# multicom-toolbox/Chromosome3D

Measured on AMD Instinct MI355X. Metric: SA-steps/sec (replica-steps/s, 20 replicas of chr1_500kb in all: 20 per GPU, weak scaling; regions of 20 steps inside the first 2172 of the schedule's 5172: MD and FIRE steps in front of the final minimisation); wall-clock per chromosome, higher is better.
Workload: dtype f32

## Files before the change

chromosome3d_amd/csrc/c3d_batch_main.cpp:

```cpp
#include <dirent.h>
#include <sys/stat.h>

#include <algorithm>
#include <atomic>
#include <chrono>
#include <condition_variable>
#include <cstdio>
#include <cstdlib>
#include <cstring>
#include <mutex>
#include <string>
#include <thread>
#include <vector>

#include "../../include/c3d.h"

namespace {

struct Job {
    std::string path, id, chrom;
    double cost = 0;
    int device = -1, half = -1;
    bool ok = false;
    std::string summary;
};
struct Options {
    std::string out;
    double K = 11, alpha = 0.5, gtol = 1e-2;
    int final_min = 1;
    bool lbfgs = false;
    int models = 20, min_steps = 3000;
    unsigned long long seed = 82364ULL;
    bool violations = false;
};
std::mutex g_print;
bool g_timeline = false;
double g_t0 = 0;
bool g_warm = true;
bool g_pair = true;

struct XcdBroker {
    std::mutex mu;
    std::condition_variable cv;
    bool busy[2] = {false, false};
    int waiting_full = 0;
    int acquire(bool half) {
        std::unique_lock<std::mutex> lk(mu);
        if (!half) {
            ++waiting_full;
            cv.wait(lk, [&] { return !busy[0] && !busy[1]; });
            --waiting_full;
            busy[0] = busy[1] = true;
            return -1;
        }
        cv.wait(lk, [&] { return waiting_full == 0 && (!busy[0] || !busy[1]); });
        const int h = busy[0] ? 1 : 0;
        busy[h] = true;
        return h;
    }
    void release(int h) {
        { std::lock_guard<std::mutex> lk(mu); if (h < 0) busy[0] = busy[1] = false; else busy[h] = false; }
        cv.notify_all();
    }
};
double now_s() { return std::chrono::duration<double>(std::chrono::steady_clock::now().time_since_epoch()).count(); }

#define TRY(call)                                                                                  \
    do {                                                                                           \
        if ((call) != C3D_OK) { job.summary = std::string(#call) + ": " + c3d_last_error(); return false; } \
    } while (0)

bool solve_one(c3d_ctx* ctx, const Options& o, Job& job, XcdBroker& gpu) {
    const double t0 = now_s();
    const std::string dir = o.out + "/" + job.chrom;
    mkdir(dir.c_str(), 0755);
    c3d_model model;
    c3d_default_model(&model);
    TRY(c3d_set_model(ctx, &model));
    double* IF = nullptr;
    int n = 0, R = 0;
    TRY(c3d_parse_if_file(job.path.c_str(), &IF, &n));
    std::vector<double> if_copy(IF, IF + (size_t)n * n);
    c3d_free(IF);
    if (n > C3D_MAX_BEADS_DEFAULT && n <= C3D_MAX_BEADS_LIMIT) TRY(c3d_set_option(ctx, "max_beads", n));
    TRY(c3d_set_if_matrix(ctx, if_copy.data(), n, o.alpha, o.K));
    const double t_k1 = now_s();
    std::vector<int32_t> d10((size_t)n * n);
    TRY(c3d_get_dist10(ctx, d10.data()));
    const std::string tbl = dir + "/contact.tbl";
    TRY(c3d_write_front_half(d10.data(), n, model.min_sep, (dir + "/" + job.id + ".dist").c_str(), (dir + "/" + job.id + ".rr").c_str(),
                             tbl.c_str(), &R));
    {
        FILE* fa = fopen((dir + "/" + job.id + ".fasta").c_str(), "w");
        if (!fa) { job.summary = "cannot write " + job.id + ".fasta"; return false; }
        fprintf(fa, ">%s\n%s\n", job.id.c_str(), std::string((size_t)n, 'M').c_str());
        if (fclose(fa) != 0) { job.summary = "cannot write " + job.id + ".fasta"; return false; }
    }
    std::vector<c3d_stage> stages(c3d_default_schedule(nullptr, 0, o.min_steps));
    c3d_default_schedule(stages.data(), (int)stages.size(), o.min_steps);
    if (o.lbfgs) stages.back().kind = 8;
    c3d_fire_params fire;
    c3d_default_fire(&fire);
    TRY(c3d_set_option(ctx, "final_minimiser", o.final_min));
    TRY(c3d_set_schedule(ctx, stages.data(), (int)stages.size(), &fire, (float)o.gtol, 250));
    bool half = false;
    if (g_pair && n <= 270) {
        TRY(c3d_set_option(ctx, "cluster_xcd_base", 0));
        TRY(c3d_set_option(ctx, "cluster_xcd_count", 4));
        TRY(c3d_init_replicas(ctx, o.models, o.seed, 0));
        double ok = 0;
        c3d_get_stat(ctx, "cluster_ok", &ok);
        half = ok != 0;
    }
    if (!half) {
        TRY(c3d_set_option(ctx, "cluster_xcd_base", 0));
        TRY(c3d_set_option(ctx, "cluster_xcd_count", 8));
        TRY(c3d_init_replicas(ctx, o.models, o.seed, 0));
    }
    const double t_front = now_s();
    double t_anneal0 = t_front;
    {
        struct Hold {
            XcdBroker& b; int h;
            ~Hold() { b.release(h); }
        } hold{gpu, gpu.acquire(half)};
        if (half) TRY(c3d_set_option(ctx, "cluster_xcd_base", 4 * hold.h));
        t_anneal0 = now_s();
        TRY(c3d_run(ctx));
        job.half = half ? hold.h : -1;
    }
    const double t_run = now_s();
    double ms = 0;
    long steps = 0, launches = 0;
    c3d_last_timing(ctx, &ms, &steps, &launches);
    const int M = o.models;
    std::vector<float> xyz((size_t)M * n * 3);
    std::vector<double> en((size_t)M * 3), rho(M);
    std::vector<int32_t> rank(M);
    TRY(c3d_get_coords(ctx, xyz.data()));
    TRY(c3d_get_energies(ctx, en.data()));
    TRY(c3d_rank(ctx, rank.data()));
    std::vector<int32_t> sats(M);
    std::vector<double> devs(M);
    TRY(c3d_score_replicas(ctx, if_copy.data(), 3, sats.data(), devs.data(), rho.data()));
    const double t_score = now_s();
    const int Rt = R;
    struct FileCloser {
        FILE* f;
        ~FileCloser() { if (f) fclose(f); }
    } lgc{fopen((o.out + "/" + job.chrom + ".log").c_str(), "w")};
    FILE* const lg = lgc.f;
    if (!lg) { job.summary = "cannot write the log"; return false; }
    fprintf(lg, "L          : %d\nRestraints : %d lines in tbl file\n\nNOE_SATISFIED(+-0.5A)  SUM_OF_DEVIATIONS>= 0.2  PDB\n", n, R);
    std::vector<std::string> names(M);
    std::vector<int32_t> vri, vrj, vrt;
    remove((dir + "/model_info.log").c_str());
    for (int k = M - 1; k >= 0; --k) {
        const int r = rank[k];
        char name[96];
        snprintf(name, sizeof name, "%s_%d.pdb", job.id.c_str(), r + 1);
        names[r] = dir + "/" + name;
        TRY(c3d_write_pdb(names[r].c_str(), xyz.data() + (size_t)r * n * 3, n, en[3 * r], en[3 * r + 1], en[3 * r + 2], name));
        int sat = sats[r];
        double dev = devs[r];
        if (o.violations) {
            if (vri.empty()) {
                int32_t *pi = nullptr, *pj = nullptr, *pt = nullptr;
                int Rr = 0;
                TRY(c3d_read_tbl(tbl.c_str(), &pi, &pj, &pt, &Rr));
                vri.assign(pi, pi + Rr); vrj.assign(pj, pj + Rr); vrt.assign(pt, pt + Rr);
                c3d_free(pi); c3d_free(pj); c3d_free(pt);
                remove((dir + "/contact_violation.txt").c_str());
            }
            TRY(c3d_write_violations(xyz.data() + (size_t)r * n * 3, n, (int)vri.size(), vri.data(), vrj.data(), vrt.data(), 0.5, ("./" + std::string(name)).c_str(),
                                     "contact.tbl", (dir + "/contact_violation.txt").c_str(), &sat, &dev));
        }
        char cnt[48], sd[48];
        snprintf(cnt, sizeof cnt, "%d/%d", sat, Rt);
        snprintf(sd, sizeof sd, "%.2f", dev);
        std::string base(name);
        base.resize(base.size() - 4);
        fprintf(lg, "%-9s             %-9s                %-25s\n", cnt, sd, base.c_str());
    }
    for (int k = M - 1; k >= 0; --k) TRY(c3d_shape_pdb(names[rank[k]].c_str(), names[rank[k]].c_str(), (dir + "/model_info.log").c_str()));
    fprintf(lg, "\n");
    for (int k = 0; k < M && k < 5; ++k) {
        char dst[96];
        snprintf(dst, sizeof dst, "%s_model%d.pdb", job.id.c_str(), k + 1);
        fprintf(lg, "model%d.pdb <= %s\n", k + 1, names[rank[k]].c_str());
        if (rename(names[rank[k]].c_str(), (dir + "/" + dst).c_str()) != 0) { job.summary = "rename failed"; return false; }
    }
    lgc.f = nullptr;
    if (fclose(lg) != 0) { job.summary = "cannot write the log"; return false; }
    char buf[512];
    const double t_end = now_s();
    snprintf(buf, sizeof buf, "%-14s N=%4d R=%6d  %2d models  best: replica %2d  E_noe %12.1f  Spearman(IF,1/d) %.4f  anneal %6.1f ms (%ld steps)  "
                              "end-to-end %.2f s  GPU %d%s  [phases: parse+K1 %.3f, front-half files+start structures %.3f, anneal %.3f, read-back+rank+Spearman %.3f, "
                              "PDB+assessment+shaping %.3f s]",
             job.chrom.c_str(), n, R, M, rank[0] + 1, en[3 * rank[0]], -rho[rank[0]], ms, steps, t_end - t0, job.device, job.half < 0 ? "" : (job.half ? " XCDs 4-7" : " XCDs 0-3"), t_k1 - t0, t_front - t_k1,
             t_run - t_anneal0, t_score - t_run, t_end - t_score);
    job.summary = buf;
    if (g_timeline) {
        std::lock_guard<std::mutex> lk(g_print);
        fprintf(stderr, "timeline %-12s N=%4d start %.4f parsed+K1 %.4f front %.4f got-GPU %.4f annealed %.4f scored %.4f end %.4f%s\n", job.chrom.c_str(), n,
                t0 - g_t0, t_k1 - g_t0, t_front - g_t0, t_anneal0 - g_t0, t_run - g_t0, t_score - g_t0, t_end - g_t0, job.half < 0 ? "" : (job.half ? " half 1" : " half 0"));
    }
    return true;
}

void collect(const std::string& arg, const std::string& pattern, std::vector<Job>& jobs) {
    struct stat st;
    if (stat(arg.c_str(), &st) != 0) { fprintf(stderr, "c3d_batch: %s not found\n", arg.c_str()); exit(2); }
    std::vector<std::string> files;
    if (S_ISDIR(st.st_mode)) {
        DIR* d = opendir(arg.c_str());
        while (dirent* e = d ? readdir(d) : nullptr) {
            const std::string f = e->d_name;
            if (f.size() > 11 && f.compare(f.size() - 11, 11, "_matrix.txt") == 0) files.push_back(arg + "/" + f);
        }
        if (d) closedir(d);
    } else {
        files.push_back(arg);
    }
    std::sort(files.begin(), files.end());
    for (const std::string& f : files) {
        if (!pattern.empty() && f.find(pattern) == std::string::npos) continue;
        Job j;
        j.path = f;
        std::string base = f.substr(f.find_last_of('/') + 1);
        j.id = base.size() > 4 && base.compare(base.size() - 4, 4, ".txt") == 0 ? base.substr(0, base.size() - 4) : base;
        j.chrom = j.id.size() > 7 && j.id.compare(j.id.size() - 7, 7, "_matrix") == 0 ? j.id.substr(0, j.id.size() - 7) : j.id;
        stat(f.c_str(), &st);
        j.cost = (double)st.st_size;
        jobs.push_back(j);
    }
}

}

int main(int argc, char** argv) {
    setenv("HSA_DISABLE_COREDUMP_ON_EXCEPTION", "1", 0);
    Options o;
    std::vector<std::string> inputs;
    std::string pattern;
    int devices = -1, lanes = 3, map_to = -1;
    for (int a = 1; a < argc; ++a) {
        const std::string s = argv[a];
        auto next = [&](const char* what) -> const char* {
            if (a + 1 >= argc) { fprintf(stderr, "c3d_batch: %s needs a value\n", what); exit(2); }
            return argv[++a];
        };
        if (s == "--out" || s == "-o") o.out = next("--out");
        else if (s == "--devices") devices = atoi(next("--devices"));
        else if (s == "--pair") g_pair = atoi(next("--pair")) != 0;
        else if (s == "--order") g_warm = std::string(next("--order")) != "lpt";
        else if (s == "--map-devices-to") map_to = atoi(next("--map-devices-to"));
        else if (s == "--lanes") lanes = std::max(1, std::min(8, atoi(next("--lanes"))));
        else if (s == "-m") o.models = atoi(next("-m"));
        else if (s == "-k") o.K = atof(next("-k"));
        else if (s == "-a") o.alpha = atof(next("-a"));
        else if (s == "--seed") o.seed = strtoull(next("--seed"), nullptr, 10);
        else if (s == "--min-steps") o.min_steps = atoi(next("--min-steps"));
        else if (s == "--gtol") o.gtol = atof(next("--gtol"));
        else if (s == "--final-minimiser") o.final_min = atoi(next("--final-minimiser"));
        else if (s == "--lbfgs") o.lbfgs = true;
        else if (s == "--pattern") pattern = next("--pattern");
        else if (s == "--violations") o.violations = true;
        else if (s == "-h" || s == "--help") { printf("usage: c3d_batch <dir | matrix files...> --out <root> [--devices N] [--lanes 3] [-m 20] [-k 11] [-a 0.5] [--seed S] [--min-steps 3000] [--gtol 1e-2] [--final-minimiser 1] [--lbfgs] [--pattern text] [--violations] [--pair 1] [--order warm|lpt] [--map-devices-to P (rehearsal)]\n"); return 0; }
        else inputs.push_back(s);
    }
    if (o.out.empty() || inputs.empty() || o.models < 1) { fprintf(stderr, "c3d_batch: need input matrices and --out <root> (see --help)\n"); return 2; }
    std::vector<Job> jobs;
    for (const std::string& in : inputs) collect(in, pattern, jobs);
    if (jobs.empty()) { fprintf(stderr, "c3d_batch: no *_matrix.txt found\n"); return 2; }
    const int ndev = c3d_device_count();
    if (ndev < 1) { fprintf(stderr, "c3d_batch: no HIP device visible: libc3d has no CPU fallback\n"); return 1; }
    if (map_to >= ndev) { fprintf(stderr, "c3d_batch: --map-devices-to %d: this machine has %d device(s)\n", map_to, ndev); return 2; }
    if (map_to >= 0) { if (devices < 1) devices = 1; if (devices > 64) devices = 64; }
    else if (devices < 1 || devices > ndev) devices = ndev;
    mkdir(o.out.c_str(), 0755);
    std::vector<size_t> order(jobs.size());
    for (size_t k = 0; k < order.size(); ++k) order[k] = k;
    std::stable_sort(order.begin(), order.end(), [&](size_t a, size_t b) { return jobs[a].cost > jobs[b].cost; });
    std::vector<double> load(devices, 0.0);
    std::vector<std::vector<size_t>> mine(devices);
    for (size_t k : order) {
        const int g = (int)(std::min_element(load.begin(), load.end()) - load.begin());
        jobs[k].device = g;
        load[g] += jobs[k].cost;
        mine[g].push_back(k);
    }
    if (g_warm && lanes > 1)
        for (int g = 0; g < devices; ++g) {
            std::vector<size_t>& q = mine[g];
            const size_t small = std::min((size_t)(lanes - 1), q.size() > 1 ? q.size() - 1 : 0);
            if (small == 0) continue;
            std::vector<size_t> head(1, q[0]);
            for (size_t k = 0; k < small; ++k) head.push_back(q[q.size() - 1 - k]);
            head.insert(head.end(), q.begin() + 1, q.end() - small);
            q.swap(head);
        }
    const double t0 = now_s();
    g_t0 = t0;
    g_timeline = getenv("C3D_BATCH_TIMELINE") != nullptr;
    std::atomic<int> failed{0};
    std::vector<std::thread> workers;
    std::vector<XcdBroker> gpu_mu(devices);
    std::vector<std::atomic<size_t>> next_job(devices);
    std::vector<std::atomic<int>> lanes_up(devices);
    for (int g = 0; g < devices; ++g) { next_job[g] = 0; lanes_up[g] = 0; }
    for (int g = 0; g < devices; ++g)
      for (int lane = 0; lane < lanes; ++lane)
        workers.emplace_back([&, g]() {
            c3d_ctx* ctx = nullptr;
            const int phys = map_to >= 0 ? map_to : g;
            if (c3d_create(phys, &ctx) != C3D_OK) {
                std::lock_guard<std::mutex> lk(g_print);
                fprintf(stderr, "c3d_batch: GPU %d: %s\n", g, c3d_last_error());
                return;
            }
            ++lanes_up[g];
            if (g_timeline) { std::lock_guard<std::mutex> lk(g_print); fprintf(stderr, "timeline lane of GPU %d has its context at %.4f\n", g, now_s() - g_t0); }
            for (;;) {
                const size_t at = next_job[g]++;
                if (at >= mine[g].size()) break;
                Job& job = jobs[mine[g][at]];
                job.ok = solve_one(ctx, o, job, gpu_mu[map_to >= 0 ? 0 : g]);
                std::lock_guard<std::mutex> lk(g_print);
                if (job.ok) printf("%s\n", job.summary.c_str());
                else { printf("FAILED: %s (%s)\n", job.chrom.c_str(), job.summary.c_str()); ++failed; }
                fflush(stdout);
            }
            c3d_destroy(ctx);
        });
    for (std::thread& w : workers) w.join();
    for (int g = 0; g < devices; ++g) {
        if (lanes_up[g] > 0) continue;
        for (size_t at = 0; at < mine[g].size(); ++at) {
            printf("FAILED: %s (no context on GPU %d)\n", jobs[mine[g][at]].chrom.c_str(), g);
            ++failed;
        }
    }
    printf("c3d_batch: %zu matrices x %d models on %d GPU(s), %d lane(s) each, in %.2f s, %d failed; models under %s/<chromosome>/<ID>_model1..5.pdb\n", jobs.size(),
           o.models, devices, lanes, now_s() - t0, failed.load(), o.out.c_str());
    return failed.load() ? 1 : 0;
}
```

chromosome3d_amd/csrc/c3d_solve_main.cpp:

```cpp
#include <sys/stat.h>

#include <chrono>
#include <cstdio>
#include <cstdlib>
#include <cstring>
#include <string>
#include <vector>

#include "../../include/c3d.h"

static void usage() {
    fprintf(stderr,
            "usage: c3d_solve (--if <IF matrix> | --tbl <contact.tbl> --n <beads>) --out <dir> [--id <ID>]\n"
            "                 [-k <K=11>] [-a <alpha=0.5>] [-m <models=20>] [--seed <82364>] [--first-replica <0>]\n"
            "                 [--device <0>] [--min-steps <3000>] [--gtol <1e-2>] [--final-minimiser <1>] [--lbfgs] [--embed] [--no-graph] [--quiet]\n"
            "                 [--precision <32>   64: anneal with the fp64 step kernels (the reference's arithmetic; with --lbfgs the final stage is\n"
            "                                     L-BFGS in fp64); beyond 2560 beads the fp64 target matrix takes 8 n^2 bytes more]\n"
            "                 [--embed-max-beads <4549>   the largest matrix --embed takes, up to 16384 (memory: 8 n^2 bytes + 4 n^2 per replica of a batch)]\n"
            "                 [--seq <one-letter residue codes | @fasta file>   residue names of the models (default: all MET)]\n"
            "                 [--similarity <path>   after the solve, the replicas against one another: one row `a b spearman rmsd` per ordered pair of\n"
            "                                        replica ids (Spearman and scaled RMSD of the pair distances, computed on the device)]\n"
            "                 [--accepted   also write <ID>a_<k>.pdb beside every <ID>_<k>.pdb, as CNS does for structures it accepts]\n");
}

#define CHECK(call)                                                              \
    do {                                                                         \
        int rc__ = (call);                                                       \
        if (rc__ != C3D_OK) {                                                    \
            fprintf(stderr, "c3d_solve: %s failed (%d): %s\n", #call, rc__, c3d_last_error()); \
            return fail_exit(out_dir);                                           \
        }                                                                        \
    } while (0)

static int fail_exit(const std::string& out_dir) {
    if (!out_dir.empty()) {
        const std::string a = out_dir + "/iam.running", b = out_dir + "/iam.failed";
        if (rename(a.c_str(), b.c_str()) != 0) { FILE* f = fopen(b.c_str(), "w"); if (f) fclose(f); }
    }
    fprintf(stderr, "ERROR! Final structures not found!\nC3D FAILED!\n");
    return 1;
}

static double now_s() { return std::chrono::duration<double>(std::chrono::steady_clock::now().time_since_epoch()).count(); }

int main(int argc, char** argv) {
    setenv("HSA_DISABLE_COREDUMP_ON_EXCEPTION", "1", 0);
    const double t_start = now_s();
    std::string if_path, tbl_path, out_dir, id, seq_arg, similarity_path;
    double K = 11, alpha = 0.5, gtol = 1e-2;
    int final_min = 1;
    int lbfgs = 0;
    int models = 20, device = 0, n_beads = 0, min_steps = 3000, use_graph = 1, quiet = 0, embed = 0, embed_max_beads = 0, accepted = 0, precision = 32;
    unsigned long long seed = 82364ULL;
    unsigned first_rep = 0;
    for (int a = 1; a < argc; ++a) {
        const std::string s = argv[a];
        auto next = [&](const char* what) -> const char* {
            if (a + 1 >= argc) { fprintf(stderr, "c3d_solve: %s needs a value\n", what); exit(2); }
            return argv[++a];
        };
        if (s == "--if" || s == "-i" || s == "-if") if_path = next("--if");
        else if (s == "--tbl") tbl_path = next("--tbl");
        else if (s == "--n") n_beads = atoi(next("--n"));
        else if (s == "--out" || s == "-o") out_dir = next("--out");
        else if (s == "--id") id = next("--id");
        else if (s == "-k") K = atof(next("-k"));
        else if (s == "-a") alpha = atof(next("-a"));
        else if (s == "-m") models = atoi(next("-m"));
        else if (s == "--seed") seed = strtoull(next("--seed"), nullptr, 10);
        else if (s == "--first-replica") first_rep = (unsigned)strtoul(next("--first-replica"), nullptr, 10);
        else if (s == "--device") device = atoi(next("--device"));
        else if (s == "--min-steps") min_steps = atoi(next("--min-steps"));
        else if (s == "--gtol") gtol = atof(next("--gtol"));
        else if (s == "--final-minimiser") final_min = atoi(next("--final-minimiser"));
        else if (s == "--lbfgs") lbfgs = 1;
        else if (s == "--embed") embed = 1;
        else if (s == "--embed-max-beads") embed_max_beads = atoi(next("--embed-max-beads"));
        else if (s == "--precision") precision = atoi(next("--precision"));
        else if (s == "--no-graph") use_graph = 0;
        else if (s == "--quiet") quiet = 1;
        else if (s == "--accepted") accepted = 1;
        else if (s == "--seq") seq_arg = next("--seq");
        else if (s == "--similarity") similarity_path = next("--similarity");
        else if (s == "-h" || s == "--help") { usage(); return 0; }
        else { fprintf(stderr, "c3d_solve: unknown option %s\n", s.c_str()); usage(); return 2; }
    }
    if (out_dir.empty() || (if_path.empty() == tbl_path.empty()) || models < 1) { usage(); return 2; }
    if (id.empty()) {
        std::string base = if_path.empty() ? std::string("model") : if_path.substr(if_path.find_last_of('/') + 1);
        if (base.size() > 4 && base.substr(base.size() - 4) == ".txt") base.resize(base.size() - 4);
        id = base;
    }
    if (!seq_arg.empty()) {
        std::string letters = seq_arg;
        if (seq_arg[0] == '@') {
            FILE* f = fopen(seq_arg.c_str() + 1, "r");
            if (!f) { fprintf(stderr, "c3d_solve: cannot read %s\n", seq_arg.c_str() + 1); return 2; }
            letters.clear();
            char line[4096];
            while (fgets(line, sizeof line, f)) if (line[0] != '>') letters += line;
            fclose(f);
        }
        c3d_set_residue_sequence(letters.c_str());
    }
    mkdir(out_dir.c_str(), 0755);
    { FILE* f = fopen((out_dir + "/iam.running").c_str(), "w"); if (!f) { fprintf(stderr, "c3d_solve: cannot write into %s\n", out_dir.c_str()); return 1; } fclose(f); }
    remove((out_dir + "/iam.failed").c_str());

    c3d_ctx* ctx = nullptr;
    CHECK(c3d_create(device, &ctx));
    const double t_ctx = now_s();
    c3d_model model;
    c3d_default_model(&model);
    CHECK(c3d_set_model(ctx, &model));

    int n = 0, R = 0;
    std::vector<int32_t> ri, rj, rt;
    double* IF = nullptr;
    if (!if_path.empty()) {
        CHECK(c3d_parse_if_file(if_path.c_str(), &IF, &n));
        if (n > C3D_MAX_BEADS_DEFAULT && n <= C3D_MAX_BEADS_LIMIT) CHECK(c3d_set_option(ctx, "max_beads", n));
        CHECK(c3d_set_if_matrix(ctx, IF, n, alpha, K));
        std::vector<int32_t> d10((size_t)n * n);
        CHECK(c3d_get_dist10(ctx, d10.data()));
        CHECK(c3d_write_front_half(d10.data(), n, model.min_sep, (out_dir + "/" + id + ".dist").c_str(),
                                   (out_dir + "/" + id + ".rr").c_str(), (out_dir + "/contact.tbl").c_str(), &R));
        if (!quiet) printf("L          : %d\nRestraints : %d lines in tbl file\n", n, R);
    } else {
        int32_t *pi = nullptr, *pj = nullptr, *pt = nullptr;
        CHECK(c3d_read_tbl(tbl_path.c_str(), &pi, &pj, &pt, &R));
        ri.assign(pi, pi + R); rj.assign(pj, pj + R); rt.assign(pt, pt + R);
        c3d_free(pi); c3d_free(pj); c3d_free(pt);
        n = n_beads;
        for (int k = 0; k < R; ++k) { if (ri[k] > n) n = ri[k]; if (rj[k] > n) n = rj[k]; }
        if (n > C3D_MAX_BEADS_DEFAULT && n <= C3D_MAX_BEADS_LIMIT) CHECK(c3d_set_option(ctx, "max_beads", n));
        CHECK(c3d_set_restraints(ctx, n, R, ri.data(), rj.data(), rt.data()));
    }

    const double t_front = now_s();
    std::vector<c3d_stage> stages(c3d_default_schedule(nullptr, 0, min_steps));
    c3d_default_schedule(stages.data(), (int)stages.size(), min_steps);
    if (lbfgs) stages.back().kind = 8;
    c3d_fire_params fire;
    c3d_default_fire(&fire);
    CHECK(c3d_set_option(ctx, "final_minimiser", final_min));
    CHECK(c3d_set_schedule(ctx, stages.data(), (int)stages.size(), &fire, (float)gtol, 250));
    CHECK(c3d_set_option(ctx, "use_graph", use_graph));
    if (precision != 32) {
        if (lbfgs) CHECK(c3d_set_option(ctx, "f64_lbfgs", 1));
        CHECK(c3d_set_option(ctx, "precision", precision));
        if (n > C3D_F64_MAX_BEADS_DEFAULT && n <= C3D_F64_MAX_BEADS_LIMIT) CHECK(c3d_set_option(ctx, "f64_max_beads", n));
    }
    CHECK(c3d_init_replicas(ctx, models, seed, first_rep));
    if (embed_max_beads) CHECK(c3d_set_option(ctx, "embed_max_beads", embed_max_beads));
    if (embed) CHECK(c3d_embed_replicas(ctx, 50));
    CHECK(c3d_run(ctx));
    const double t_run = now_s();

    std::vector<float> xyz((size_t)models * n * 3);
    std::vector<double> en((size_t)models * 3);
    CHECK(c3d_get_coords(ctx, xyz.data()));
    CHECK(c3d_get_energies(ctx, en.data()));
    for (int r = 0; r < models; ++r) {
        char name[64];
        snprintf(name, sizeof name, "%s_%u.pdb", id.c_str(), first_rep + (unsigned)r + 1u);
        CHECK(c3d_write_pdb((out_dir + "/" + name).c_str(), xyz.data() + (size_t)r * n * 3, n, en[3 * r], en[3 * r + 1],
                            en[3 * r + 2], name));
        if (accepted) {
            snprintf(name, sizeof name, "%sa_%u.pdb", id.c_str(), first_rep + (unsigned)r + 1u);
            CHECK(c3d_write_pdb((out_dir + "/" + name).c_str(), xyz.data() + (size_t)r * n * 3, n, en[3 * r], en[3 * r + 1],
                                en[3 * r + 2], name));
        }
    }
    if (!similarity_path.empty()) {
        std::vector<double> rho((size_t)models * models), rmsd((size_t)models * models);
        CHECK(c3d_compare_replicas(ctx, nullptr, 0, rho.data(), rmsd.data()));
        FILE* f = fopen(similarity_path.c_str(), "w");
        if (!f) { fprintf(stderr, "c3d_solve: cannot write %s\n", similarity_path.c_str()); return fail_exit(out_dir); }
        fprintf(f, "# replica_a replica_b spearman rmsd   (pair distances of a scaled onto b's; replica r is %s_<r+1>.pdb)\n", id.c_str());
        for (int a = 0; a < models; ++a)
            for (int b = 0; b < models; ++b)
                if (a != b) fprintf(f, "%u %u %.5f %.5f\n", first_rep + (unsigned)a, first_rep + (unsigned)b, rho[(size_t)a * models + b], rmsd[(size_t)a * models + b]);
        fclose(f);
    }
    double ms = 0;
    long steps = 0, launches = 0;
    c3d_last_timing(ctx, &ms, &steps, &launches);
    if (!quiet) {
        printf(accepted ? "trial and accepted structures written.\n" : "trial structures written.\n");
        printf("c3d_solve: %d beads, %d restraints, %d models, %ld SA steps/model in %.1f ms on device %d (%.3g replica-steps/s)\n",
               n, R, models, steps, ms, device, ms > 0 ? 1e3 * (double)steps * models / ms : 0.0);
        if (IF) {
            std::vector<double> rho(models);
            if (c3d_score_replicas(ctx, IF, 3, nullptr, nullptr, rho.data()) == C3D_OK)
                for (int r = 0; r < models; ++r)
                    printf("  model %2u  E_noe %14.2f  Spearman(IF,d) %.4f\n", first_rep + r + 1, en[3 * r], rho[r]);
            else fprintf(stderr, "c3d_solve: models not scored: %s\n", c3d_last_error());
        }
    }
    if (!quiet)
        printf("c3d_solve wall: device init %.3f s, parse + K1 + front-half files %.3f s, anneal (incl. graph build) %.3f s, "
               "read-back + PDB + scoring %.3f s, total %.3f s\n", t_ctx - t_start, t_front - t_ctx, t_run - t_front, now_s() - t_run,
               now_s() - t_start);
    if (IF) c3d_free(IF);
    c3d_destroy(ctx);
    remove((out_dir + "/iam.running").c_str());
    return 0;
}
```

Measured before the change: 4.736 million.

## Overlap host-side parsing, front-half file writes and PDB output with GPU work

Adds a small host task pool and look-ahead parser so the interaction matrix is parsed ahead of time, the front-half files (.dist/.rr/.tbl/.fasta) are written on a helper thread while annealing runs, and per-model PDB writing and shape analysis run in parallel. The goal is to hide host I/O and parsing latency behind device work and each other. The metric counts replica-steps per second inside the annealing phase, so host-side overlap may not affect it, and the extra threads add scheduling complexity and more error-handling paths.

```diff
diff --git a/chromosome3d_amd/csrc/c3d_batch_main.cpp b/chromosome3d_amd/csrc/c3d_batch_main.cpp
--- a/chromosome3d_amd/csrc/c3d_batch_main.cpp
+++ b/chromosome3d_amd/csrc/c3d_batch_main.cpp
@@ -8,12 +8,15 @@
 #include <cstdio>
 #include <cstdlib>
 #include <cstring>
+#include <future>
+#include <memory>
 #include <mutex>
 #include <string>
 #include <thread>
 #include <vector>
 
 #include "../../include/c3d.h"
+#include "c3d_overlap.h"
 
 namespace {
 
@@ -32,6 +35,7 @@
     int models = 20, min_steps = 3000;
     unsigned long long seed = 82364ULL;
     bool violations = false;
+    int host_threads = 8;
 };
 std::mutex g_print;
 bool g_timeline = false;
@@ -69,32 +73,79 @@
     do {                                                                                           \
         if ((call) != C3D_OK) { job.summary = std::string(#call) + ": " + c3d_last_error(); return false; } \
     } while (0)
-
-bool solve_one(c3d_ctx* ctx, const Options& o, Job& job, XcdBroker& gpu) {
+#define STEP(err, call) ((call) == C3D_OK ? true : ((err) = std::string(#call) + ": " + c3d_last_error(), false))
+
+struct Parsed {
+    std::unique_ptr<double, void (*)(void*)> IF{nullptr, c3d_free};
+    int n = 0;
+    std::string err;
+    double t_begin = 0, t_end = 0;
+};
+Parsed parse_job(const Job& job) {
+    Parsed out;
+    out.t_begin = now_s();
+    double* IF = nullptr;
+    int n = 0;
+    if (STEP(out.err, c3d_parse_if_file(job.path.c_str(), &IF, &n))) { out.IF.reset(IF); out.n = n; }
+    out.t_end = now_s();
+    return out;
+}
+
+struct FrontFiles {
+    int R = 0;
+    std::string err;
+    double t_begin = 0, t_end = 0;
+};
+FrontFiles write_front_files(const Job& job, const std::string& dir, const std::string& tbl, const c3d_model& model, const std::vector<int32_t>& d10, int n) {
+    FrontFiles out;
+    out.t_begin = now_s();
+    int R = 0;
+    if (STEP(out.err, c3d_write_front_half(d10.data(), n, model.min_sep, (dir + "/" + job.id + ".dist").c_str(), (dir + "/" + job.id + ".rr").c_str(),
+                                          tbl.c_str(), &R))) {
+        FILE* fa = fopen((dir + "/" + job.id + ".fasta").c_str(), "w");
+        if (!fa) out.err = "cannot write " + job.id + ".fasta";
+        else {
+            fprintf(fa, ">%s\n%s\n", job.id.c_str(), std::string((size_t)n, 'M').c_str());
+            if (fclose(fa) != 0) out.err = "cannot write " + job.id + ".fasta";
+        }
+    }
+    out.R = R;
+    out.t_end = now_s();
+    return out;
+}
+
+struct Lane {
+    c3d_overlap::TaskPool pool;
+    explicit Lane(int helpers) : pool(helpers) {}
+};
+
+bool solve_body(c3d_ctx* ctx, const Options& o, Job& job, XcdBroker& gpu, Lane& lane, c3d_overlap::LookAhead<Parsed>& matrices, size_t at,
+                std::future<FrontFiles>& front) {
     const double t0 = now_s();
     const std::string dir = o.out + "/" + job.chrom;
     mkdir(dir.c_str(), 0755);
     c3d_model model;
     c3d_default_model(&model);
     TRY(c3d_set_model(ctx, &model));
-    double* IF = nullptr;
-    int n = 0, R = 0;
-    TRY(c3d_parse_if_file(job.path.c_str(), &IF, &n));
-    std::vector<double> if_copy(IF, IF + (size_t)n * n);
-    c3d_free(IF);
+    const Parsed parsed = matrices.take(at);
+    const double t_taken = now_s();
+    if (!parsed.err.empty()) { job.summary = parsed.err; return false; }
+    const int n = parsed.n;
+    const double* const if_copy = parsed.IF.get();
+    int R = 0;
     if (n > C3D_MAX_BEADS_DEFAULT && n <= C3D_MAX_BEADS_LIMIT) TRY(c3d_set_option(ctx, "max_beads", n));
-    TRY(c3d_set_if_matrix(ctx, if_copy.data(), n, o.alpha, o.K));
+    TRY(c3d_set_if_matrix(ctx, if_copy, n, o.alpha, o.K));
     const double t_k1 = now_s();
-    std::vector<int32_t> d10((size_t)n * n);
-    TRY(c3d_get_dist10(ctx, d10.data()));
+    const auto d10 = std::make_shared<std::vector<int32_t>>((size_t)n * n);
+    TRY(c3d_get_dist10(ctx, d10->data()));
+    const double t_d10 = now_s();
     const std::string tbl = dir + "/contact.tbl";
-    TRY(c3d_write_front_half(d10.data(), n, model.min_sep, (dir + "/" + job.id + ".dist").c_str(), (dir + "/" + job.id + ".rr").c_str(),
-                             tbl.c_str(), &R));
-    {
-        FILE* fa = fopen((dir + "/" + job.id + ".fasta").c_str(), "w");
-        if (!fa) { job.summary = "cannot write " + job.id + ".fasta"; return false; }
-        fprintf(fa, ">%s\n%s\n", job.id.c_str(), std::string((size_t)n, 'M').c_str());
-        if (fclose(fa) != 0) { job.summary = "cannot write " + job.id + ".fasta"; return false; }
+    front = lane.pool.submit([&job, dir, tbl, model, d10, n] { return write_front_files(job, dir, tbl, model, *d10, n); });
+    FrontFiles files;
+    if (lane.pool.size() == 0) {
+        files = front.get();
+        if (!files.err.empty()) { job.summary = files.err; return false; }
+        R = files.R;
     }
     std::vector<c3d_stage> stages(c3d_default_schedule(nullptr, 0, o.min_steps));
     c3d_default_schedule(stages.data(), (int)stages.size(), o.min_steps);
@@ -142,8 +193,14 @@
     TRY(c3d_rank(ctx, rank.data()));
     std::vector<int32_t> sats(M);
     std::vector<double> devs(M);
-    TRY(c3d_score_replicas(ctx, if_copy.data(), 3, sats.data(), devs.data(), rho.data()));
+    TRY(c3d_score_replicas(ctx, if_copy, 3, sats.data(), devs.data(), rho.data()));
     const double t_score = now_s();
+    if (front.valid()) {
+        files = front.get();
+        if (!files.err.empty()) { job.summary = files.err; return false; }
+        R = files.R;
+    }
+    const double t_joined = now_s();
     const int Rt = R;
     struct FileCloser {
         FILE* f;
@@ -155,12 +212,7 @@
     std::vector<std::string> names(M);
     std::vector<int32_t> vri, vrj, vrt;
     remove((dir + "/model_info.log").c_str());
-    for (int k = M - 1; k >= 0; --k) {
-        const int r = rank[k];
-        char name[96];
-        snprintf(name, sizeof name, "%s_%d.pdb", job.id.c_str(), r + 1);
-        names[r] = dir + "/" + name;
-        TRY(c3d_write_pdb(names[r].c_str(), xyz.data() + (size_t)r * n * 3, n, en[3 * r], en[3 * r + 1], en[3 * r + 2], name));
+    auto table_row = [&](int r, const char* name) -> bool {
         int sat = sats[r];
         double dev = devs[r];
         if (o.violations) {
@@ -181,8 +233,58 @@
         std::string base(name);
         base.resize(base.size() - 4);
         fprintf(lg, "%-9s             %-9s                %-25s\n", cnt, sd, base.c_str());
-    }
-    for (int k = M - 1; k >= 0; --k) TRY(c3d_shape_pdb(names[rank[k]].c_str(), names[rank[k]].c_str(), (dir + "/model_info.log").c_str()));
+        return true;
+    };
+    if (lane.pool.size() == 0) {
+        for (int k = M - 1; k >= 0; --k) {
+            const int r = rank[k];
+            char name[96];
+            snprintf(name, sizeof name, "%s_%d.pdb", job.id.c_str(), r + 1);
+            names[r] = dir + "/" + name;
+            TRY(c3d_write_pdb(names[r].c_str(), xyz.data() + (size_t)r * n * 3, n, en[3 * r], en[3 * r + 1], en[3 * r + 2], name));
+            if (!table_row(r, name)) return false;
+        }
+        for (int k = M - 1; k >= 0; --k) TRY(c3d_shape_pdb(names[rank[k]].c_str(), names[rank[k]].c_str(), (dir + "/model_info.log").c_str()));
+    } else {
+        for (int r = 0; r < M; ++r) {
+            char name[96];
+            snprintf(name, sizeof name, "%s_%d.pdb", job.id.c_str(), r + 1);
+            names[r] = dir + "/" + name;
+        }
+        std::vector<std::string> werr(M), serr(M);
+        auto drop_parts = [&] { for (int r = 0; r < M; ++r) remove((names[r] + ".info").c_str()); };
+        std::string terr;
+        int t_at = -1;
+        {
+            c3d_overlap::IndexRun models(lane.pool, M, 8, [&](int idx) {
+                const int k = M - 1 - idx;
+                const int r = rank[k];
+                const char* name = names[r].c_str() + dir.size() + 1;
+                if (!STEP(werr[k], c3d_write_pdb(names[r].c_str(), xyz.data() + (size_t)r * n * 3, n, en[3 * r], en[3 * r + 1], en[3 * r + 2], name))) return;
+                const std::string part = names[r] + ".info";
+                remove(part.c_str());
+                if (c3d_shape_pdb(names[r].c_str(), names[r].c_str(), part.c_str()) != C3D_OK)
+                    serr[k] = std::string("c3d_shape_pdb(names[rank[k]].c_str(), names[rank[k]].c_str(), (dir + \"/model_info.log\").c_str()): ") + c3d_last_error();
+            });
+            for (int k = M - 1; k >= 0; --k)
+                if (!table_row(rank[k], names[rank[k]].c_str() + dir.size() + 1)) { terr = job.summary; t_at = k; break; }
+            models.finish();
+        }
+        std::string first;
+        for (int k = M - 1; k >= 0 && first.empty(); --k) first = !werr[k].empty() ? werr[k] : k == t_at ? terr : std::string();
+        for (int k = M - 1; k >= 0 && first.empty(); --k) first = serr[k];
+        if (!first.empty()) { drop_parts(); job.summary = first; return false; }
+        FILE* info = fopen((dir + "/model_info.log").c_str(), "a");
+        if (!info) { drop_parts(); job.summary = "c3d_shape_pdb: cannot append to " + dir + "/model_info.log"; return false; }
+        for (int k = M - 1; k >= 0; --k) {
+            FILE* pf = fopen((names[rank[k]] + ".info").c_str(), "rb");
+            char buf[4096];
+            for (size_t got; pf && (got = fread(buf, 1, sizeof buf, pf)) > 0;) fwrite(buf, 1, got, info);
+            if (pf) fclose(pf);
+        }
+        fclose(info);
+        drop_parts();
+    }
     fprintf(lg, "\n");
     for (int k = 0; k < M && k < 5; ++k) {
         char dst[96];
@@ -202,10 +304,22 @@
     job.summary = buf;
     if (g_timeline) {
         std::lock_guard<std::mutex> lk(g_print);
-        fprintf(stderr, "timeline %-12s N=%4d start %.4f parsed+K1 %.4f front %.4f got-GPU %.4f annealed %.4f scored %.4f end %.4f%s\n", job.chrom.c_str(), n,
-                t0 - g_t0, t_k1 - g_t0, t_front - g_t0, t_anneal0 - g_t0, t_run - g_t0, t_score - g_t0, t_end - g_t0, job.half < 0 ? "" : (job.half ? " half 1" : " half 0"));
+        fprintf(stderr, "timeline %-12s N=%4d start %.4f parsed+K1 %.4f front %.4f got-GPU %.4f annealed %.4f scored %.4f end %.4f%s"
+                        "  [parse %.4f .. %.4f, matrix taken %.4f, set-matrix %.4f, d10 %.4f, front files %.4f .. %.4f, joined %.4f, job %.4f s]\n", job.chrom.c_str(), n,
+                t0 - g_t0, t_k1 - g_t0, t_front - g_t0, t_anneal0 - g_t0, t_run - g_t0, t_score - g_t0, t_end - g_t0, job.half < 0 ? "" : (job.half ? " half 1" : " half 0"),
+                parsed.t_begin - g_t0, parsed.t_end - g_t0, t_taken - g_t0, t_k1 - g_t0, t_d10 - g_t0, files.t_begin - g_t0, files.t_end - g_t0, t_joined - g_t0, t_end - t0);
     }
     return true;
+}
+
+bool solve_one(c3d_ctx* ctx, const Options& o, Job& job, XcdBroker& gpu, Lane& lane, c3d_overlap::LookAhead<Parsed>& matrices, size_t at) {
+    std::future<FrontFiles> front;
+    const bool ok = solve_body(ctx, o, job, gpu, lane, matrices, at, front);
+    if (front.valid()) {
+        const FrontFiles files = front.get();
+        if (!files.err.empty()) job.summary = files.err;
+    }
+    return ok;
 }
 
 void collect(const std::string& arg, const std::string& pattern, std::vector<Job>& jobs) {
@@ -240,6 +354,7 @@
 
 int main(int argc, char** argv) {
     setenv("HSA_DISABLE_COREDUMP_ON_EXCEPTION", "1", 0);
+    const double t_main = now_s();
     Options o;
     std::vector<std::string> inputs;
     std::string pattern;
@@ -266,22 +381,29 @@
         else if (s == "--lbfgs") o.lbfgs = true;
         else if (s == "--pattern") pattern = next("--pattern");
         else if (s == "--violations") o.violations = true;
-        else if (s == "-h" || s == "--help") { printf("usage: c3d_batch <dir | matrix files...> --out <root> [--devices N] [--lanes 3] [-m 20] [-k 11] [-a 0.5] [--seed S] [--min-steps 3000] [--gtol 1e-2] [--final-minimiser 1] [--lbfgs] [--pattern text] [--violations] [--pair 1] [--order warm|lpt] [--map-devices-to P (rehearsal)]\n"); return 0; }
+        else if (s == "--host-threads") o.host_threads = std::max(1, std::min(64, atoi(next("--host-threads"))));
+        else if (s == "-h" || s == "--help") { printf("usage: c3d_batch <dir | matrix files...> --out <root> [--devices N] [--lanes 3] [-m 20] [-k 11] [-a 0.5] [--seed S] [--min-steps 3000] [--gtol 1e-2] [--final-minimiser 1] [--lbfgs] [--pattern text] [--violations] [--pair 1] [--order warm|lpt] [--host-threads 8 (1: no helper threads)] [--map-devices-to P (rehearsal)]\n"); return 0; }
         else inputs.push_back(s);
     }
     if (o.out.empty() || inputs.empty() || o.models < 1) { fprintf(stderr, "c3d_batch: need input matrices and --out <root> (see --help)\n"); return 2; }
     std::vector<Job> jobs;
     for (const std::string& in : inputs) collect(in, pattern, jobs);
     if (jobs.empty()) { fprintf(stderr, "c3d_batch: no *_matrix.txt found\n"); return 2; }
+    std::vector<size_t> order(jobs.size());
+    for (size_t k = 0; k < order.size(); ++k) order[k] = k;
+    std::stable_sort(order.begin(), order.end(), [&](size_t a, size_t b) { return jobs[a].cost > jobs[b].cost; });
+    const bool overlap = o.host_threads > 1;
+    const size_t head_job = order[0];
+    std::future<Parsed> head;
+    if (overlap) head = std::async(std::launch::async, [&jobs, head_job] { return parse_job(jobs[head_job]); });
+    const double t_args = now_s();
     const int ndev = c3d_device_count();
+    const double t_count = now_s();
     if (ndev < 1) { fprintf(stderr, "c3d_batch: no HIP device visible: libc3d has no CPU fallback\n"); return 1; }
     if (map_to >= ndev) { fprintf(stderr, "c3d_batch: --map-devices-to %d: this machine has %d device(s)\n", map_to, ndev); return 2; }
     if (map_to >= 0) { if (devices < 1) devices = 1; if (devices > 64) devices = 64; }
     else if (devices < 1 || devices > ndev) devices = ndev;
     mkdir(o.out.c_str(), 0755);
-    std::vector<size_t> order(jobs.size());
-    for (size_t k = 0; k < order.size(); ++k) order[k] = k;
-    std::stable_sort(order.begin(), order.end(), [&](size_t a, size_t b) { return jobs[a].cost > jobs[b].cost; });
     std::vector<double> load(devices, 0.0);
     std::vector<std::vector<size_t>> mine(devices);
     for (size_t k : order) {
@@ -303,6 +425,16 @@
     const double t0 = now_s();
     g_t0 = t0;
     g_timeline = getenv("C3D_BATCH_TIMELINE") != nullptr;
+    if (g_timeline) fprintf(stderr, "timeline main: arguments and job list %.4f s, device count (first runtime call) %.4f s, queues %.4f s; executor starts %.4f s after main\n",
+                            t_args - t_main, t_count - t_args, t0 - t_count, t0 - t_main);
+    const int helpers = overlap ? std::max(1, std::min(7, o.host_threads / lanes - 1)) : 0;
+    std::vector<std::unique_ptr<c3d_overlap::LookAhead<Parsed>>> matrices;
+    for (int g = 0; g < devices; ++g)
+        matrices.emplace_back(new c3d_overlap::LookAhead<Parsed>(mine[g].size(), (size_t)lanes, overlap ? lanes : 0, [&, g](size_t at) {
+            const size_t j = mine[g][at];
+            if (j == head_job && head.valid()) return head.get();
+            return parse_job(jobs[j]);
+        }));
     std::atomic<int> failed{0};
     std::vector<std::thread> workers;
     std::vector<XcdBroker> gpu_mu(devices);
@@ -312,6 +444,7 @@
     for (int g = 0; g < devices; ++g)
       for (int lane = 0; lane < lanes; ++lane)
         workers.emplace_back([&, g]() {
+            Lane lane_state(helpers);
             c3d_ctx* ctx = nullptr;
             const int phys = map_to >= 0 ? map_to : g;
             if (c3d_create(phys, &ctx) != C3D_OK) {
@@ -325,7 +458,7 @@
                 const size_t at = next_job[g]++;
                 if (at >= mine[g].size()) break;
                 Job& job = jobs[mine[g][at]];
-                job.ok = solve_one(ctx, o, job, gpu_mu[map_to >= 0 ? 0 : g]);
+                job.ok = solve_one(ctx, o, job, gpu_mu[map_to >= 0 ? 0 : g], lane_state, *matrices[g], at);
                 std::lock_guard<std::mutex> lk(g_print);
                 if (job.ok) printf("%s\n", job.summary.c_str());
                 else { printf("FAILED: %s (%s)\n", job.chrom.c_str(), job.summary.c_str()); ++failed; }
@@ -334,6 +467,7 @@
             c3d_destroy(ctx);
         });
     for (std::thread& w : workers) w.join();
+    matrices.clear();
     for (int g = 0; g < devices; ++g) {
         if (lanes_up[g] > 0) continue;
         for (size_t at = 0; at < mine[g].size(); ++at) {
diff --git a/chromosome3d_amd/csrc/c3d_overlap.h b/chromosome3d_amd/csrc/c3d_overlap.h
--- /dev/null
+++ b/chromosome3d_amd/csrc/c3d_overlap.h
@@ -0,0 +1,138 @@
+#pragma once
+
+#include <algorithm>
+#include <atomic>
+#include <condition_variable>
+#include <deque>
+#include <functional>
+#include <future>
+#include <memory>
+#include <mutex>
+#include <optional>
+#include <thread>
+#include <type_traits>
+#include <utility>
+#include <vector>
+
+namespace c3d_overlap {
+
+class TaskPool {
+  public:
+    explicit TaskPool(int threads) {
+        for (int t = 0; t < threads; ++t) workers_.emplace_back([this] { work(); });
+    }
+    TaskPool(const TaskPool&) = delete;
+    TaskPool& operator=(const TaskPool&) = delete;
+    ~TaskPool() {
+        { std::lock_guard<std::mutex> lk(mu_); stop_ = true; }
+        cv_.notify_all();
+        for (std::thread& w : workers_) w.join();
+    }
+    int size() const { return (int)workers_.size(); }
+
+    template <class F>
+    auto submit(F&& fn) -> std::future<std::invoke_result_t<std::decay_t<F>&>> {
+        using R = std::invoke_result_t<std::decay_t<F>&>;
+        auto task = std::make_shared<std::packaged_task<R()>>(std::forward<F>(fn));
+        std::future<R> fut = task->get_future();
+        if (workers_.empty()) { (*task)(); return fut; }
+        { std::lock_guard<std::mutex> lk(mu_); queue_.emplace_back([task] { (*task)(); }); }
+        cv_.notify_one();
+        return fut;
+    }
+
+  private:
+    void work() {
+        for (;;) {
+            std::function<void()> fn;
+            {
+                std::unique_lock<std::mutex> lk(mu_);
+                cv_.wait(lk, [&] { return stop_ || !queue_.empty(); });
+                if (queue_.empty()) return;
+                fn = std::move(queue_.front());
+                queue_.pop_front();
+            }
+            fn();
+        }
+    }
+    std::mutex mu_;
+    std::condition_variable cv_;
+    std::deque<std::function<void()>> queue_;
+    bool stop_ = false;
+    std::vector<std::thread> workers_;
+};
+
+class IndexRun {
+  public:
+    IndexRun(TaskPool& pool, int count, int max_threads, std::function<void(int)> fn) : count_(count), fn_(std::move(fn)) {
+        const int helpers = std::max(0, std::min(std::min(count, max_threads) - 1, pool.size()));
+        for (int h = 0; h < helpers; ++h) done_.push_back(pool.submit([this] { drain(); }));
+    }
+    IndexRun(const IndexRun&) = delete;
+    IndexRun& operator=(const IndexRun&) = delete;
+    ~IndexRun() { finish(); }
+    void finish() {
+        drain();
+        for (std::future<void>& d : done_) d.get();
+        done_.clear();
+    }
+
+  private:
+    void drain() { for (int i; (i = next_.fetch_add(1)) < count_;) fn_(i); }
+    const int count_;
+    const std::function<void(int)> fn_;
+    std::atomic<int> next_{0};
+    std::vector<std::future<void>> done_;
+};
+
+template <class T>
+class LookAhead {
+  public:
+    LookAhead(size_t total, size_t window, int threads, std::function<T(size_t)> produce)
+        : total_(total), window_(window < 1 ? 1 : window), produce_(std::move(produce)), slots_(total) {
+        for (int t = 0; t < threads; ++t) producers_.emplace_back([this] { work(); });
+    }
+    LookAhead(const LookAhead&) = delete;
+    LookAhead& operator=(const LookAhead&) = delete;
+    ~LookAhead() {
+        { std::lock_guard<std::mutex> lk(mu_); stop_ = true; }
+        cv_.notify_all();
+        for (std::thread& p : producers_) p.join();
+    }
+    T take(size_t i) {
+        if (producers_.empty()) return produce_(i);
+        std::unique_lock<std::mutex> lk(mu_);
+        ++takes_;
+        cv_.notify_all();
+        cv_.wait(lk, [&] { return slots_[i].has_value(); });
+        T v = std::move(*slots_[i]);
+        slots_[i].reset();
+        return v;
+    }
+
+  private:
+    void work() {
+        for (;;) {
+            size_t i;
+            {
+                std::unique_lock<std::mutex> lk(mu_);
+                cv_.wait(lk, [&] { return stop_ || next_ >= total_ || next_ < takes_ + window_; });
+                if (stop_ || next_ >= total_) return;
+                i = next_++;
+            }
+            T v = produce_(i);
+            { std::lock_guard<std::mutex> lk(mu_); slots_[i].emplace(std::move(v)); }
+            cv_.notify_all();
+        }
+    }
+    const size_t total_, window_;
+    const std::function<T(size_t)> produce_;
+    std::mutex mu_;
+    std::condition_variable cv_;
+    std::vector<std::optional<T>> slots_;
+    size_t next_ = 0, takes_ = 0;
+    bool stop_ = false;
+    std::vector<std::thread> producers_;
+};
+
+}
diff --git a/chromosome3d_amd/csrc/c3d_solve_main.cpp b/chromosome3d_amd/csrc/c3d_solve_main.cpp
--- a/chromosome3d_amd/csrc/c3d_solve_main.cpp
+++ b/chromosome3d_amd/csrc/c3d_solve_main.cpp
@@ -4,10 +4,13 @@
 #include <cstdio>
 #include <cstdlib>
 #include <cstring>
+#include <future>
+#include <memory>
 #include <string>
 #include <vector>
 
 #include "../../include/c3d.h"
+#include "c3d_overlap.h"
 
 static void usage() {
     fprintf(stderr,
@@ -20,6 +23,7 @@
             "                 [--seq <one-letter residue codes | @fasta file>   residue names of the models (default: all MET)]\n"
             "                 [--similarity <path>   after the solve, the replicas against one another: one row `a b spearman rmsd` per ordered pair of\n"
             "                                        replica ids (Spearman and scaled RMSD of the pair distances, computed on the device)]\n"
+            "                 [--host-threads <8>   host threads for the host-only phases (parse, front-half files, model files); 1: one after the other]\n"
             "                 [--accepted   also write <ID>a_<k>.pdb beside every <ID>_<k>.pdb, as CNS does for structures it accepts]\n");
 }
 
@@ -32,6 +36,20 @@
         }                                                                        \
     } while (0)
 
+struct Outcome {
+    int rc = C3D_OK;
+    std::string what;
+};
+#define OUTCOME(o, call)                                                        \
+    do {                                                                        \
+        (o).rc = (call);                                                        \
+        if ((o).rc != C3D_OK) (o).what = std::string(#call) + " failed (" + std::to_string((o).rc) + "): " + c3d_last_error(); \
+    } while (0)
+#define CHECK_OUTCOME(o)                                                        \
+    do {                                                                        \
+        if ((o).rc != C3D_OK) { fprintf(stderr, "c3d_solve: %s\n", (o).what.c_str()); return fail_exit(out_dir); } \
+    } while (0)
+
 static int fail_exit(const std::string& out_dir) {
     if (!out_dir.empty()) {
         const std::string a = out_dir + "/iam.running", b = out_dir + "/iam.failed";
@@ -51,6 +69,7 @@
     int final_min = 1;
     int lbfgs = 0;
     int models = 20, device = 0, n_beads = 0, min_steps = 3000, use_graph = 1, quiet = 0, embed = 0, embed_max_beads = 0, accepted = 0, precision = 32;
+    int host_threads = 8;
     unsigned long long seed = 82364ULL;
     unsigned first_rep = 0;
     for (int a = 1; a < argc; ++a) {
@@ -81,6 +100,7 @@
         else if (s == "--quiet") quiet = 1;
         else if (s == "--accepted") accepted = 1;
         else if (s == "--seq") seq_arg = next("--seq");
+        else if (s == "--host-threads") host_threads = atoi(next("--host-threads"));
         else if (s == "--similarity") similarity_path = next("--similarity");
         else if (s == "-h" || s == "--help") { usage(); return 0; }
         else { fprintf(stderr, "c3d_solve: unknown option %s\n", s.c_str()); usage(); return 2; }
@@ -107,6 +127,19 @@
     { FILE* f = fopen((out_dir + "/iam.running").c_str(), "w"); if (!f) { fprintf(stderr, "c3d_solve: cannot write into %s\n", out_dir.c_str()); return 1; } fclose(f); }
     remove((out_dir + "/iam.failed").c_str());
 
+    c3d_overlap::TaskPool pool(host_threads > 1 ? std::min(7, host_threads - 1) : 0);
+    struct ParsedIF { Outcome o; double* IF = nullptr; int n = 0; };
+    std::future<ParsedIF> parsing;
+    auto parse_if = [&if_path] {
+        ParsedIF p;
+        double* IF = nullptr;
+        int n = 0;
+        OUTCOME(p.o, c3d_parse_if_file(if_path.c_str(), &IF, &n));
+        p.IF = IF; p.n = n;
+        return p;
+    };
+    if (!if_path.empty() && pool.size() > 0) parsing = pool.submit(parse_if);
+
     c3d_ctx* ctx = nullptr;
     CHECK(c3d_create(device, &ctx));
     const double t_ctx = now_s();
@@ -117,15 +150,33 @@
     int n = 0, R = 0;
     std::vector<int32_t> ri, rj, rt;
     double* IF = nullptr;
+    struct FrontFiles { Outcome o; int R = 0; };
+    std::future<FrontFiles> front;
     if (!if_path.empty()) {
-        CHECK(c3d_parse_if_file(if_path.c_str(), &IF, &n));
+        {
+            const ParsedIF p = parsing.valid() ? parsing.get() : parse_if();
+            CHECK_OUTCOME(p.o);
+            IF = p.IF; n = p.n;
+        }
         if (n > C3D_MAX_BEADS_DEFAULT && n <= C3D_MAX_BEADS_LIMIT) CHECK(c3d_set_option(ctx, "max_beads", n));
         CHECK(c3d_set_if_matrix(ctx, IF, n, alpha, K));
-        std::vector<int32_t> d10((size_t)n * n);
-        CHECK(c3d_get_dist10(ctx, d10.data()));
-        CHECK(c3d_write_front_half(d10.data(), n, model.min_sep, (out_dir + "/" + id + ".dist").c_str(),
-                                   (out_dir + "/" + id + ".rr").c_str(), (out_dir + "/contact.tbl").c_str(), &R));
-        if (!quiet) printf("L          : %d\nRestraints : %d lines in tbl file\n", n, R);
+        const auto d10p = std::make_shared<std::vector<int32_t>>((size_t)n * n);
+        CHECK(c3d_get_dist10(ctx, d10p->data()));
+        front = pool.submit([d10p, n, model, out_dir, id] {
+            FrontFiles f;
+            const std::vector<int32_t>& d10 = *d10p;
+            int R = 0;
+            OUTCOME(f.o, c3d_write_front_half(d10.data(), n, model.min_sep, (out_dir + "/" + id + ".dist").c_str(),
+                                              (out_dir + "/" + id + ".rr").c_str(), (out_dir + "/contact.tbl").c_str(), &R));
+            f.R = R;
+            return f;
+        });
+        if (pool.size() == 0) {
+            const FrontFiles f = front.get();
+            CHECK_OUTCOME(f.o);
+            R = f.R;
+            if (!quiet) printf("L          : %d\nRestraints : %d lines in tbl file\n", n, R);
+        }
     } else {
         int32_t *pi = nullptr, *pj = nullptr, *pt = nullptr;
         CHECK(c3d_read_tbl(tbl_path.c_str(), &pi, &pj, &pt, &R));
@@ -156,21 +207,32 @@
     if (embed) CHECK(c3d_embed_replicas(ctx, 50));
     CHECK(c3d_run(ctx));
     const double t_run = now_s();
+    if (front.valid()) {
+        const FrontFiles f = front.get();
+        CHECK_OUTCOME(f.o);
+        R = f.R;
+        if (!quiet) printf("L          : %d\nRestraints : %d lines in tbl file\n", n, R);
+    }
 
     std::vector<float> xyz((size_t)models * n * 3);
     std::vector<double> en((size_t)models * 3);
     CHECK(c3d_get_coords(ctx, xyz.data()));
     CHECK(c3d_get_energies(ctx, en.data()));
-    for (int r = 0; r < models; ++r) {
-        char name[64];
-        snprintf(name, sizeof name, "%s_%u.pdb", id.c_str(), first_rep + (unsigned)r + 1u);
-        CHECK(c3d_write_pdb((out_dir + "/" + name).c_str(), xyz.data() + (size_t)r * n * 3, n, en[3 * r], en[3 * r + 1],
-                            en[3 * r + 2], name));
-        if (accepted) {
+    {
+        std::vector<Outcome> wrote(models);
+        c3d_overlap::IndexRun files(pool, models, 8, [&](int r) {
+            Outcome& o = wrote[r];
+            char name[64];
+            snprintf(name, sizeof name, "%s_%u.pdb", id.c_str(), first_rep + (unsigned)r + 1u);
+            OUTCOME(o, c3d_write_pdb((out_dir + "/" + name).c_str(), xyz.data() + (size_t)r * n * 3, n, en[3 * r], en[3 * r + 1],
+                                     en[3 * r + 2], name));
+            if (o.rc != C3D_OK || !accepted) return;
             snprintf(name, sizeof name, "%sa_%u.pdb", id.c_str(), first_rep + (unsigned)r + 1u);
-            CHECK(c3d_write_pdb((out_dir + "/" + name).c_str(), xyz.data() + (size_t)r * n * 3, n, en[3 * r], en[3 * r + 1],
-                                en[3 * r + 2], name));
-        }
+            OUTCOME(o, c3d_write_pdb((out_dir + "/" + name).c_str(), xyz.data() + (size_t)r * n * 3, n, en[3 * r], en[3 * r + 1],
+                                     en[3 * r + 2], name));
+        });
+        files.finish();
+        for (int r = 0; r < models; ++r) CHECK_OUTCOME(wrote[r]);
     }
     if (!similarity_path.empty()) {
         std::vector<double> rho((size_t)models * models), rmsd((size_t)models * models);
```

Result: slower. 4.666 million (-1.5%).
